# plancherb1/parallel-DDP

Measured on AMD Instinct MI355X. Metric: DDP iterations/sec (Kuka iiwa14 N=128, 8 alphas, 4 shooting segments), higher is better.
Workload: dtype f32; 1 GPU; BASELINE configs[2]: Kuka iiwa14 RBD (n=14,m=7), N=128, 8 alphas x 4 shooting segments, Euler, fp32, joint cost, T=0.5 s, WAFR example inputs + N(0,1e-3) velocity noise; problems_per_gpu=16384, problems_total=16384, hipgraph=True, cost_to_go_slots_written=all, handle_options=library defaults

## Files before the change

### parallel-ddp_amd/csrc/bp_mfma.hpp

```cpp
#pragma once

#include <hip/hip_runtime.h>

#include "ab_compact.hpp"
#include "solver_state.hpp"

#ifndef PDDP_MX_EXP
#define PDDP_MX_EXP 0
#endif

#ifndef PDDP_MX_STAGE_K
#define PDDP_MX_STAGE_K 0
#endif
#ifndef PDDP_MX_DMA_MASK
#define PDDP_MX_DMA_MASK 0
#endif
#ifndef PDDP_MX_ORDER
#define PDDP_MX_ORDER 0
#endif
#ifndef PDDP_MX_GJ
#define PDDP_MX_GJ 0
#endif

namespace pddp {
// ... 382 lines not shown
    asm volatile(
        "s_mov_b32 m0, %[l0]\n\ts_nop 0\n\tbuffer_load_dword %[v], %[dab], %[s0] offen lds\n\t"
        "s_mov_b32 m0, %[l1]\n\ts_nop 0\n\tbuffer_load_dword %[v], %[dab], %[s1] offen lds\n\t"
        "s_mov_b32 m0, %[l2]\n\ts_nop 0\n\tbuffer_load_dword %[v], %[dab], %[s2] offen lds\n\t"
        "s_mov_b32 %[keep], exec_hi\n\ts_mov_b32 exec_hi, 0\n\ts_mov_b32 m0, %[l3]\n\ts_nop 0\n\tbuffer_load_dword %[v], %[dg], %[sg] offen lds\n\t"
        "s_mov_b32 exec_hi, %[keep]"
        : [keep] "=&s"(keep)
        : [l0] "s"(l0), [l1] "s"(l0 + 4u * kMxDmaRegion), [l2] "s"(l0 + 8u * kMxDmaRegion), [l3] "s"(l0 + 12u * kMxDmaRegion), [v] "v"(lane4), [dab] "s"(dab), [dg] "s"(dg),
          [s0] "s"(s0), [s1] "s"(s1), [s2] "s"(s2), [sg] "s"(sg)
        : "memory", "m0");
#endif
    if constexpr (HQQ)
        asm volatile("s_mov_b32 m0, %[l4]\n\ts_nop 0\n\tbuffer_load_dword %[v], %[dh], %[sh] offen lds" :: [l4] "s"(l0 + 16u * kMxDmaRegion), [v] "v"(lane4), [dh] "s"(dh), [sh] "s"(sh) : "memory", "m0");
}
template <bool FS>
__device__ __forceinline__ void mx_lds_knot(MxKnotIn<float, FS, true>& k, unsigned half, unsigned aA, unsigned aB, unsigned aT, unsigned aG, int g, int c, int ub, float dt) {
    constexpr int NX = 14, NU = 7;
    typedef const float __attribute__((address_space(3))) * lptr;
    const int u0 = 2 * g, sc = mx_state<float>(c);
    const bool cx = sc < NX, cu = ub < NU, c14 = (sc == NX), g3 = g < 3;
    const lptr pA = (lptr)(size_t)(aA + half), pB = (lptr)(size_t)(aB + half), pT = (lptr)(size_t)(aT + half), pG = (lptr)(size_t)(aG + half);
    const float ta0 = pA[0], ta1 = pA[1], tb0 = pB[0], tb1 = pB[1];
    k.A0[0] = cx ? ((sc == u0) ? 1.f : ((sc == u0 + 7) ? dt : 0.f)) : 0.f;
    k.A0[1] = (cx && g3) ? ((sc == u0 + 1) ? 1.f : ((sc == u0 + 8) ? dt : 0.f)) : 0.f;
    k.A0[2] = cx ? ta0 : 0.f; k.A0[3] = (cx && g3) ? ta1 : 0.f;
    k.B1[0] = 0.f; k.B1[1] = 0.f;
    k.B1[2] = cu ? tb0 : 0.f; k.B1[3] = (cu && g3) ? tb1 : 0.f;
    if (FS) {
        const float t0 = pT[0], t1 = pT[7];
        k.BT0 = (cx && sc >= 7) ? t0 : 0.f; k.BT1 = (cx && sc >= 7 && u0 + 1 < NU) ? t1 : 0.f;
    }
    const float gx[4] = {pG[0], pG[1], pG[7], pG[8]};
    const float gu0 = pG[NX], gu1 = pG[NX + 1];
#pragma unroll
    for (int r = 0; r < 4; r++) k.CXX[r] = (c14 && (g3 || !(r & 1))) ? gx[r] : 0.f;
    k.CUX0 = c14 ? gu0 : 0.f; k.CUX1 = (c14 && u0 + 1 < NU) ? gu1 : 0.f;
    k.hx = 0.f; k.hu = 0.f;
}

__device__ __forceinline__ void mx_store_gain_pieces(const mx_u4& w, __amdgpu_buffer_rsrc_t rKT, __amdgpu_buffer_rsrc_t rdu, int lane, unsigned knot) {
    const unsigned soK = knot * (unsigned)(14 * 7 * 4), sod = knot * (unsigned)(7 * 4);
    if (lane < 24) __builtin_amdgcn_raw_buffer_store_b128(w, rKT, 16u * (unsigned)lane, soK, 0);
    else if (lane == 24) { mx_u2 h; h[0] = w[0]; h[1] = w[1]; __builtin_amdgcn_raw_buffer_store_b64(h, rKT, 384u, soK, 0); }
    else if (lane == 25) __builtin_amdgcn_raw_buffer_store_b128(w, rdu, 0u, sod, 0);
    else if (lane == 26) { mx_u3 t; t[0] = w[0]; t[1] = w[1]; t[2] = w[2]; __builtin_amdgcn_raw_buffer_store_b96(t, rdu, 16u, sod, 0); }
}
constexpr int kMxGainStores = 4, kMxCtgStores = 3;
constexpr int kMxKeepP = 1, kMxFuseSweep = 2, kMxLds = 400, kMxDmaFloats = 2 * 5 * 64 + 256 + 112;
template <typename T, bool FS, bool DIAGH, bool CAB, bool FUSE, bool HQQ = false>
__device__ void arm_mx_bp_block(T* lds, const Buffers<T>& b, const Dims& dm, int pb, int blk, T hq1, T hq2, T hr, T dt, int flags) {
    static_assert(!HQQ || DIAGH, "the compact position block rides on the diagonal-Hessian path");
    using X = Mx<T>;
    using mx4 = mx4t<T>;
    const int keepP = flags & kMxKeepP;
    const bool fuse = FUSE && blk < dm.M - 1;
    constexpr int NX = 14, NU = 7, NM = 21, SZP = NX * NX, SZAB = NX * NM, SZH = NM * NM;
    const int lane = threadIdx.x & 63, g = lane >> 4, c = lane & 15, u0 = 2 * g, sc = mx_state<T>(c);
    const int cg = X::g_of(c), cr = X::r_of(c);
    const int ub = (cr < 2) ? 2 * cg + cr : 8;
    const SolverState<T>& st = b.state[pb];
    if (st.done) return;
    const int N = dm.N, NBk = dm.NB;
    const T rho = st.rho;
    const size_t halfP = (size_t)(b.Pp - b.P), halfp = (size_t)(b.pp - b.p), knot0 = (size_t)pb * N;
    T* Pw = b.P + (st.pw ? halfP : 0) + knot0 * SZP;
    const T* Pr = b.P + (st.pw ? 0 : halfP) + knot0 * SZP;
    T* pw = b.p + (st.pw ? halfp : 0) + knot0 * NX;
    const T* pr = b.p + (st.pw ? 0 : halfp) + knot0 * NX;
    const T* AB = b.AB + knot0 * SZAB; const T* H = b.H + knot0 * SZH; const T* gg = b.g + knot0 * NM;
    T* KT = b.KT + knot0 * (NX * NU); T* du = b.du + knot0 * NU; T* ApBK = b.ApBK + knot0 * SZP; T* Bdu = b.Bdu + knot0 * NX;
    const T* dcur = b.dcur + knot0 * NX;
    const T* xc = b.xb + ((size_t)pb * 2 + st.cur) * N * NX; const T* xp2 = b.xb + ((size_t)pb * 2 + st.cur2) * N * NX;
    const bool cx = sc < NX, cu = ub < NU, c14 = (sc == NX);
    bool diag[4];
#pragma unroll
    for (int r = 0; r < 4; r++) diag[r] = (X::q_of(g, r) == c);

    int ks = NBk * (blk + 1) - 1, iterCount;
    mx4 Pa;
    if (ks == N - 1) {
        const T* Hf = H + (size_t)ks * SZH; const T* gf = gg + (size_t)ks * NM;
        Pa = mx_load_col<T>(cx ? Hf + sc * NM : gf, g, cx || c14);
        if (keepP) mx_store_col<T>(cx ? Pw + (size_t)(ks - 1) * SZP + sc * NX : pw + (size_t)(ks - 1) * NX, g, cx || c14, Pa);
        ks--; iterCount = NBk - 2;
    } else {
        iterCount = NBk - 1;
        const T* bP = Pr + (size_t)ks * SZP;
        Pa = mx_load_col<T>(bP + sc * NX, g, cx);
        if (lane < NX) {
            T dot = T(0), val = T(0);
            for (int j = 0; j < NX; j++) {
                const T pj = bP[lane + NX * j];
                dot += pj * (xc[NX * (ks + 1) + j] - xp2[NX * (ks + 1) + j]);
                val += dcur[(size_t)ks * NX + j] * pj;
            }
            lds[lane] = (dot + pr[(size_t)ks * NX + lane]) + val;
        }
        wsync();
        if (c14) {
#pragma unroll
            for (int r = 0; r < 4; r++) { const int sr = mx_state_gr(g, r); Pa[r] = (sr < NX) ? lds[sr] : T(0); }
        }
        wsync();
    }
    T dJ00 = T(0), dJ01 = T(0), dJ10 = T(0), dJ11 = T(0);
    const mx4 zero = {T(0), T(0), T(0), T(0)};
    T* ldsI = lds + 16;
// ... 317 lines not shown
```

### parallel-ddp_amd/csrc/mx_launch.hpp

```cpp
#pragma once

#include <hip/hip_runtime.h>

#include "solver_state.hpp"

namespace pddp {

template <typename T>
void launch_bp_mfma(hipStream_t s, const Buffers<T>& b, const Dims& dm, int batch, bool diag_h, T hq1, T hq2, T hr, T dt, bool keep_P, bool fuse_sweep, int ee = 0);
template <typename T>
void launch_sweep_maps(hipStream_t s, const Buffers<T>& b, const Dims& dm, int batch);

}
```

### parallel-ddp_amd/csrc/pddp_mx.hip

```cpp
#include <hip/hip_runtime.h>

#include "bp_mfma.hpp"
#include "mx_launch.hpp"

#ifdef PDDP_MX_WAVES
#define PDDP_MX_WAVES_OF(CAB, HQQ) PDDP_MX_WAVES
#else
#define PDDP_MX_WAVES_OF(CAB, HQQ) ((CAB) ? 6 : 5)
#endif

namespace pddp {

template <bool FS, bool DIAGH, bool CAB, bool FUSE, bool HQQ = false>
__global__ __launch_bounds__(64) __attribute__((amdgpu_waves_per_eu(PDDP_MX_WAVES_OF(CAB, HQQ), PDDP_MX_WAVES_OF(CAB, HQQ)))) void k_bp_mfma(Buffers<float> b, Dims dm, int batch, float hq1, float hq2, float hr, float dt, int flags) {
    __shared__ __attribute__((aligned(16))) float lds[kMxLds + kMxDmaFloats];
    const int inst = blockIdx.x;
    if (inst >= batch * dm.M) return;
    arm_mx_bp_block<float, FS, DIAGH, CAB, FUSE, HQQ>(lds, b, dm, inst / dm.M, inst % dm.M, hq1, hq2, hr, dt, flags);
}
template <bool FS, bool DIAGH, bool CAB, bool FUSE, bool HQQ = false>
__global__ __launch_bounds__(64) void k_bp_mfma_f64(Buffers<double> b, Dims dm, int batch, double hq1, double hq2, double hr, double dt, int flags) {
    __shared__ __attribute__((aligned(16))) double lds[kMxLds];
    const int inst = blockIdx.x;
    if (inst >= batch * dm.M) return;
    arm_mx_bp_block<double, FS, DIAGH, CAB, FUSE, HQQ>(lds, b, dm, inst / dm.M, inst % dm.M, hq1, hq2, hr, dt, flags);
}
__device__ __forceinline__ float mx_uniform(float v) { return __int_as_float(__builtin_amdgcn_readfirstlane(__float_as_int(v))); }
__device__ __forceinline__ double mx_uniform(double v) {
    return __hiloint2double(__builtin_amdgcn_readfirstlane(__double2hiint(v)), __builtin_amdgcn_readfirstlane(__double2loint(v)));
}
template <bool FS, bool CAB, bool FUSE, bool HQQ = false>
__global__ __launch_bounds__(64) __attribute__((amdgpu_waves_per_eu(PDDP_MX_WAVES_OF(CAB, HQQ), PDDP_MX_WAVES_OF(CAB, HQQ)))) void k_bp_mfma_pc(Buffers<float> b, Dims dm, int batch, int ee, float dt, int flags) {
    __shared__ __attribute__((aligned(16))) float lds[kMxLds + kMxDmaFloats];
    const int inst = blockIdx.x;
    if (inst >= batch * dm.M) return;
    float hq1, hq2, hr;
    cost_diag_weights_at<float>(b.cwt, ee, inst / dm.M, hq1, hq2, hr);
    arm_mx_bp_block<float, FS, true, CAB, FUSE, HQQ>(lds, b, dm, inst / dm.M, inst % dm.M, mx_uniform(hq1), mx_uniform(hq2), mx_uniform(hr), dt, flags);
}
template <bool FS, bool CAB, bool FUSE, bool HQQ = false>
__global__ __launch_bounds__(64) void k_bp_mfma_f64_pc(Buffers<double> b, Dims dm, int batch, int ee, double dt, int flags) {
    __shared__ __attribute__((aligned(16))) double lds[kMxLds];
    const int inst = blockIdx.x;
    if (inst >= batch * dm.M) return;
    double hq1, hq2, hr;
    cost_diag_weights_at<double>(b.cwt, ee, inst / dm.M, hq1, hq2, hr);
    arm_mx_bp_block<double, FS, true, CAB, FUSE, HQQ>(lds, b, dm, inst / dm.M, inst % dm.M, mx_uniform(hq1), mx_uniform(hq2), mx_uniform(hr), dt, flags);
}
template <bool FS, bool DIAGH, bool CAB, bool FUSE, bool HQQ = false>
static void launch_one(hipStream_t s, unsigned n, const Buffers<float>& b, const Dims& dm, int batch, float hq1, float hq2, float hr, float dt, int kp, int ee) {
    if constexpr (DIAGH) { if (b.cwt) { hipLaunchKernelGGL((k_bp_mfma_pc<FS, CAB, FUSE, HQQ>), dim3(n), dim3(64), 0, s, b, dm, batch, ee, dt, kp); return; } }
    hipLaunchKernelGGL((k_bp_mfma<FS, DIAGH, CAB, FUSE, HQQ>), dim3(n), dim3(64), 0, s, b, dm, batch, hq1, hq2, hr, dt, kp);
}
template <bool FS, bool DIAGH, bool CAB, bool FUSE, bool HQQ = false>
static void launch_one(hipStream_t s, unsigned n, const Buffers<double>& b, const Dims& dm, int batch, double hq1, double hq2, double hr, double dt, int kp, int ee) {
    if constexpr (DIAGH) { if (b.cwt) { hipLaunchKernelGGL((k_bp_mfma_f64_pc<FS, CAB, FUSE, HQQ>), dim3(n), dim3(64), 0, s, b, dm, batch, ee, dt, kp); return; } }
    hipLaunchKernelGGL((k_bp_mfma_f64<FS, DIAGH, CAB, FUSE, HQQ>), dim3(n), dim3(64), 0, s, b, dm, batch, hq1, hq2, hr, dt, kp);
}

template <typename T>
void launch_bp_mfma(hipStream_t s, const Buffers<T>& b, const Dims& dm, int batch, bool diag_h, T hq1, T hq2, T hr, T dt, bool keep_P, bool fuse_sweep, int ee) {
    const unsigned n = (unsigned)batch * dm.M;
    const int kp = (keep_P ? kMxKeepP : 0) | ((fuse_sweep && b.segmap) ? kMxFuseSweep : 0);
    const bool cab = b.ABc != nullptr && diag_h;
#define PDDP_MX_LAUNCH(FS, DH, CB, FU) launch_one<FS, DH, CB, FU>(s, n, b, dm, batch, hq1, hq2, hr, dt, kp, ee)
    const bool fu = (kp & kMxFuseSweep) != 0;
    if (cab && b.Hc) {
#define PDDP_MX_LAUNCH_Q(FS, FU) launch_one<FS, true, true, FU, true>(s, n, b, dm, batch, hq1, hq2, hr, dt, kp, ee)
        if (dm.M > 1) { if (fu) PDDP_MX_LAUNCH_Q(true, true); else PDDP_MX_LAUNCH_Q(true, false); }
        else PDDP_MX_LAUNCH_Q(false, false);
#undef PDDP_MX_LAUNCH_Q
        return;
    }
    if (dm.M > 1) {
        if (cab) { if (fu) PDDP_MX_LAUNCH(true, true, true, true); else PDDP_MX_LAUNCH(true, true, true, false); }
        else if (diag_h) { if (fu) PDDP_MX_LAUNCH(true, true, false, true); else PDDP_MX_LAUNCH(true, true, false, false); }
        else { if (fu) PDDP_MX_LAUNCH(true, false, false, true); else PDDP_MX_LAUNCH(true, false, false, false); }
    } else {
        if (cab) PDDP_MX_LAUNCH(false, true, true, false);
        else if (diag_h) PDDP_MX_LAUNCH(false, true, false, false);
        else PDDP_MX_LAUNCH(false, false, false, false);
    }
#undef PDDP_MX_LAUNCH
}
template void launch_bp_mfma<float>(hipStream_t, const Buffers<float>&, const Dims&, int, bool, float, float, float, float, bool, bool, int);
template void launch_bp_mfma<double>(hipStream_t, const Buffers<double>&, const Dims&, int, bool, double, double, double, double, bool, bool, int);

template <typename T, int PER>
__global__ __launch_bounds__(64) void k_sweep_maps(Buffers<T> b, Dims dm, int batch) {
    constexpr int NX = 14, W = 64 / PER;
    const int lane = threadIdx.x % W, pb = blockIdx.x * PER + threadIdx.x / W;
    if (pb >= batch) return;
    const SolverState<T>& st = b.state[pb];
    if (st.done) return;
    for (int i = 0; i < dm.M; i++) if (b.err[(size_t)pb * dm.M + i]) return;
    const int N = dm.N, NBk = dm.NB, l = lane < NX ? lane : NX - 1;
    const T* xcur = b.xb + ((size_t)pb * 2 + st.cur) * N * NX; const T* dcur = b.dcur + (size_t)pb * N * NX;
    T es = T(0), et = T(0);
    if (dm.M == 4) {
        constexpr int S = 3;
        T ph[S][NX + 1], dk[S], base[S];
#pragma unroll
        for (int sgm = 0; sgm < S; sgm++) {
            const T* o = b.segmap + ((size_t)pb * 4 + sgm) * 256;
            const int k = (sgm + 1) * NBk - 1;
#pragma unroll
            for (int cc = 0; cc <= NX; cc++) ph[sgm][cc] = o[cc * 16 + l];
            dk[sgm] = dcur[(size_t)k * NX + l]; base[sgm] = xcur[(size_t)(k + 1) * NX + l];
        }
#pragma unroll
        for (int sgm = 0; sgm < S; sgm++) {
            const int k = (sgm + 1) * NBk - 1;
            T ns = ph[sgm][NX], nt = dk[sgm];
#pragma unroll
            for (int cc = 0; cc < NX; cc++) { ns = Mx<T>::fma(ph[sgm][cc], __shfl(es, cc, W), ns); nt = Mx<T>::fma(ph[sgm][cc], __shfl(et, cc, W), nt); }
            es = ns; et = nt;
            if (lane < NX) for (int a = 0; a < dm.A; a++) b.xs[(((size_t)pb * dm.A + a) * N + k + 1) * NX + lane] = base[sgm] + (et - b.alpha[a] * es);
        }
        return;
    }
    for (int sgm = 0; sgm < dm.M - 1; sgm++) {
        const T* o = b.segmap + ((size_t)pb * dm.M + sgm) * 256;
        const int k = (sgm + 1) * NBk - 1;
        T ns = o[14 * 16 + l], nt = dcur[(size_t)k * NX + l];
#pragma unroll
        for (int cc = 0; cc < NX; cc++) {
            const T ph = o[cc * 16 + l];
            ns = Mx<T>::fma(ph, __shfl(es, cc, W), ns); nt = Mx<T>::fma(ph, __shfl(et, cc, W), nt);
        }
        es = ns; et = nt;
        if (lane < NX) {
            const T base = xcur[(size_t)(k + 1) * NX + lane];
            for (int a = 0; a < dm.A; a++) b.xs[(((size_t)pb * dm.A + a) * N + k + 1) * NX + lane] = base + (et - b.alpha[a] * es);
        }
    }
}
template <typename T>
void launch_sweep_maps(hipStream_t s, const Buffers<T>& b, const Dims& dm, int batch) {
    if (batch >= 2048) hipLaunchKernelGGL((k_sweep_maps<T, 4>), dim3((unsigned)((batch + 3) / 4)), dim3(64), 0, s, b, dm, batch);
// ... 7 lines not shown
```

### parallel-ddp_amd/csrc/solver_impl.hpp

```cpp
#pragma once
#include "solver_base.hpp"
#include "kernels.hpp"
#include "handle_setup.hpp"
#include "slots.hpp"
#include "cost_table.hpp"
#include "diag_cost_table.hpp"
#include "goal_traj_table.hpp"
#include "mpc_slots.hpp"
#include "mpc_record.hpp"
#include "tl_launch.hpp"
#include "mx_launch.hpp"

using namespace pddp;

template <typename P, int INTEG, typename T>
struct Solver : SolverBase {
    static constexpr int NX = P::NX, NU = P::NU, NM = NX + NU, NP = P::NPOS;
    Buffers<T> b{};
    MpcBuffers<T> mb{};
    T* d_xActual = nullptr; T* d_goal_in = nullptr; int* d_shift = nullptr;
    unsigned char* d_mpc_out = nullptr;
    PinnedBuf h_state;
    PinnedBuf h_stage;
    Dims dm{};
    SolverParams sp{};
    CostWeights<T> cw{};
    T dt{};
    std::map<std::string, std::pair<void*, size_t>> arrays;
    std::vector<DeviceBuf> allocs;
    template <typename Mem> int reserve(MemBuf<Mem>& buf, size_t bytes, const char* what, size_t min_cap = 0) {
        if (buf.holds(bytes)) return 0;
        if (buf.ptr) HIPCHK(hipStreamSynchronize(stream));
        return buf.reserve(bytes, min_cap) ? 0 : fail(Mem::kFailCode, what);
    }
    KernelPlan plan;
    void resolve_plan() { plan = make_kernel_plan(cfg, PlantTraits{P::PLANT, NX, NU, P::kScalarPlugin, P::kPluginCost}, sizeof(T) == 4, tl_variant); }
    int tl_variant = -1;
    T tl_grav = T(0);
    void derive_tl_model(const ArmModel<T>& hm) {
        ArmTlModel<T> m;
        tl_variant = -1;
        if (arm_tl_model_from_tables(m, hm))
            for (int v = 0; v < 2; v++) if (arm_tl_models_equal(m, arm_tl_builtin<T>(v))) tl_variant = v;
        tl_grav = hm.grav;
    }
    void derive_tl_model(const EmptyModel&) {}
    void drop_graph() override { if (graph) { hipGraphExecDestroy(graph); graph = nullptr; graph_mode = -1; } if (graph_n) { hipGraphExecDestroy(graph_n); graph_n = nullptr; } }
    int ab_view(int to_compact) override {
        if constexpr (P::PLANT == 4) {
            if (b.ABc) { launch_abc_convert<T>(stream, b, (int)(cfg.batch * cfg.N), cfg.N, dt, to_compact); HIPCHK(hipGetLastError()); HIPCHK(hipStreamSynchronize(stream)); }
        }
        return 0;
    }
    int ab_keep_reference_layout() override {
        if (!b.ABc) return 0;
        int rc = ab_view(0);
        b.ABc = nullptr; b.Hc = nullptr; drop_graph();
        return rc;
    }
    int h_view() override {
        if constexpr (P::PLANT == 4) {
            if (b.Hc) {
                hipLaunchKernelGGL((k_hc_expand<T>), dim3((cfg.batch * cfg.N + 63) / 64), dim3(64), 0, stream, b, (int)(cfg.batch * cfg.N), cfg.N, hw[1], hw[2]);
                HIPCHK(hipGetLastError()); HIPCHK(hipStreamSynchronize(stream));
            }
        }
        return 0;
    }
    int cand_view(int to_records) override {
        if constexpr (P::PLANT != 4) {
            if (b.xw && plan.cf_fp_staged) {
                const dim3 g((unsigned)(((size_t)cfg.batch * cfg.N * cfg.A + 255) / 256));
                if (to_records) hipLaunchKernelGGL((k_cand_to_xw<P, T>), g, dim3(256), 0, stream, b, dm, (int)cfg.batch);
                else hipLaunchKernelGGL((k_xw_to_cand<P, T>), g, dim3(256), 0, stream, b, dm, (int)cfg.batch);
                HIPCHK(hipGetLastError()); HIPCHK(hipStreamSynchronize(stream));
            }
        }
        cand_stale = false;
        return 0;
    }
    int reference_views(int what) override {
        if ((what & 1) && cfg.M > 1) { int rc = ab_view(0); if (rc) return rc; }
        hipLaunchKernelGGL((k_reference_views<P, T>), dim3(cfg.N, cfg.batch), dim3(64), 0, stream, b, dm, what);
        HIPCHK(hipGetLastError()); HIPCHK(hipStreamSynchronize(stream));
        if (what & 1) fs_vars_stale = false;
        if (what & 2) cand_stale = false;
        return 0;
    }
    int model_changed() override {
        typename P::Model hm;
        HIPCHK(hipMemcpy(&hm, b.model, sizeof(hm), hipMemcpyDeviceToHost));
        derive_tl_model(hm);
        resolve_plan();
        drop_graph();
        return 0;
    }
    bool mpc_used = false;
    bool lean_ctg_ran = false;
    bool keep_all_ctg() const { return !cfg.boundary_cost_to_go_only || cfg.mpc_mode || mpc_used; }
    hipGraphExec_t graph = nullptr;
    int graph_mode = -1;
    size_t fp_lds = 0;

    ~Solver() override {
        drop_graph();
        for (hipEvent_t e : trace_ev) hipEventDestroy(e);
        for (hipEvent_t e : slots_ev) if (e) hipEventDestroy(e);
        delete intake;
        if (stream && !intake_of) hipStreamDestroy(stream);
    }
    void register_model(void* dmodel, const ArmModel<T>&) {
        arrays["model_I"] = {dmodel, sizeof(T) * kArmNB * 36};
        arrays["model_F"] = {(char*)dmodel + offsetof(ArmModel<T>, F), sizeof(T) * kArmNB * 16};
    }
    void register_model(void*, const EmptyModel&) {}
    template <typename U> int alloc(const char* name, U** out, size_t count) {
        DeviceBuf blk;
        if (!blk.reserve(count * sizeof(U))) return fail(PDDP_ENOMEM, std::string("hipMalloc failed for ") + name);
        if (hipMemset(blk.ptr, 0, count * sizeof(U)) != hipSuccess) return fail(PDDP_ENODEVICE, "hipMemset failed");
        arrays[name] = {blk.ptr, count * sizeof(U)}; *out = blk.template as<U>();
        allocs.push_back(std::move(blk));
        return 0;
    }
    int init() override {
        const pddp_config& c = cfg;
        int ndev = 0;
        if (hipGetDeviceCount(&ndev) != hipSuccess || ndev <= c.device)
            return fail(PDDP_ENODEVICE, "no HIP device available: libpddp has no CPU fallback");
        HIPCHK(hipSetDevice(c.device));
#ifdef PDDP_REF_PLANT_FILE
        if constexpr (P::PLANT == 5) { const std::string complaint = ref_plugin_setup<T>(c.N); if (!complaint.empty()) return fail(PDDP_EINVAL, complaint); }
#endif
        if constexpr (P::PLANT == 5) {
            if (!scalar_plugin_qdd_is_dynamics<P, T>())
                return fail(PDDP_EINVAL, "plant 5: the plug-in's gradient routine returns a qdd that differs from its dynamics routine at the same state; the kernel families build the "
                                         "integrators' stage states from either one, so the two have to be the same numbers (call the dynamics routine inside the gradient routine)");
        }
        if (intake_of) stream = intake_of->stream;
        else HIPCHK(hipStreamCreateWithFlags(&stream, hipStreamNonBlocking));
        dm.N = c.N; dm.M = c.M; dm.A = c.A; dm.NB = c.N / c.M;
        cap_batch = c.batch;
        sp = solver_params_of(c); cw = cost_weights_of<T, P::PLANT>(c); dt = time_step<T>(c);
        const size_t B = c.batch, N = c.N, A = c.A, M = c.M;
        int rc = for_each_array<NX, NU>(c, b, mb, arrays, [this](const char* name, auto** out, size_t count) { return alloc(name, out, count); });
        if (rc) return rc;
        const MpcInputRun in = mpc_input_run(sizeof(T), NX, B);
        if ((rc = alloc("mpc_in", &d_xActual, in.elems))) return rc;
        d_goal_in = mpc_at<T>(d_xActual, in.goal); d_shift = mpc_at<int>(d_xActual, in.shift);
        arrays["xActual"] = {d_xActual, in.x_bytes}; arrays["shift"] = {d_shift, in.shift_bytes};
        std::vector<T> al(A);
        alpha_table(c, al.data());
        HIPCHK(hipMemcpy(b.alpha, al.data(), A * sizeof(T), hipMemcpyHostToDevice));
        typename P::Model hm; fill_model(hm, c);
// ... 147 lines not shown
            break;
        }
        if constexpr (P::PLANT != 4) { if (L.cand_to_xw && b.xw) hipLaunchKernelGGL((k_cand_to_xw<P, T>), dim3((unsigned)(((size_t)B * cfg.N * cfg.A + 255) / 256)), dim3(256), 0, s, b, dm, (int)B); }
    }
    T hw[3] = {T(0), T(0), T(0)};
    void note_setup_weights() { const bool ee = cfg.ee_cost != 0; hw[0] = ee ? cw.Q_xEE : cw.Q1; hw[1] = ee ? cw.Q_xdEE : cw.Q2; hw[2] = ee ? cw.R_EE : cw.R; }
    void launch_nis(hipStream_t s, int mode, int part = -1) {
        const unsigned B = cfg.batch;
        if (part == 0) return;
        note_setup_weights();
        switch (plan.nis) {
        case kNisTl:
            if constexpr (P::PLANT == 4) launch_nis_tl<T>(s, tl_variant, b, dm, cw, dt, tl_grav, mode, (int)B);
            break;
        case kNisTl7:
            if constexpr (P::PLANT == 4) launch_nis_tl7<T>(s, tl_variant, b, dm, cw, dt, tl_grav, mode, (int)B);
            break;
        case kNisLg:
            if constexpr (P::PLANT == 4) {
                if (cfg.ee_cost) hipLaunchKernelGGL((k_nis_lg<T, true>), dim3((cfg.N + 31) / 32, B), dim3(256), 0, s, b, dm, cw, dt, mode);
                else hipLaunchKernelGGL((k_nis_lg<T>), dim3((cfg.N + 31) / 32, B), dim3(256), 0, s, b, dm, cw, dt, mode);
            }
            break;
        case kNisTs:
            if constexpr (P::PLANT != 4) with_cost_plant([&](auto pl) { using Q = decltype(pl); hipLaunchKernelGGL((k_nis_ts<Q, INTEG, T>), dim3((B * cfg.N + 63) / 64), dim3(64), 0, s, b, dm, cw, dt, mode, (int)B); });
            break;
        case kNisKb:
            if constexpr (P::PLANT != 4 && P::NX + P::NU <= 16 && INTEG == 3 && P::kScalarPlugin) {
                const int units = (int)(B * cfg.N);
                with_cost_plant([&](auto pl) {
                    using Q = decltype(pl);
                    if (plan.kb_nis == 16) hipLaunchKernelGGL((k_nis_kb<Q, T, 16>), dim3((units + 15) / 16), dim3(64), 0, s, b, dm, cw, dt, mode, (int)B);
                    else if (plan.kb_nis == 20) hipLaunchKernelGGL((k_nis_kb<Q, T, 20>), dim3((units + 19) / 20), dim3(64), 0, s, b, dm, cw, dt, mode, (int)B);
                    else if (plan.kb_nis == 64 && sizeof(T) == 4) hipLaunchKernelGGL((k_nis_kb<Q, T, sizeof(T) == 4 ? 64 : 16>), dim3((units + 63) / 64), dim3(64), 0, s, b, dm, cw, dt, mode, (int)B);
                    else hipLaunchKernelGGL((k_nis_kb<Q, T, 32>), dim3((units + 31) / 32), dim3(64), 0, s, b, dm, cw, dt, mode, (int)B);
                });
            }
            break;
        case kNisGl:
            if constexpr (P::PLANT != 4 && P::NX + P::NU <= 16) {
                with_cost_plant([&](auto pl) {
                    using Q = decltype(pl);
                    if (plan.gl_nis8) hipLaunchKernelGGL((k_nis_gl<Q, INTEG, T, 8>), dim3((B * cfg.N + 7) / 8), dim3(64), 0, s, b, dm, cw, dt, mode, (int)B);
                    else hipLaunchKernelGGL((k_nis_gl<Q, INTEG, T, 16>), dim3((B * cfg.N + 3) / 4), dim3(64), 0, s, b, dm, cw, dt, mode, (int)B);
                });
            }
            break;
        case kNisCoop:
            if constexpr (P::PLANT == 4) { if (b.cwt) { hipLaunchKernelGGL((k_nis<P, INTEG, T, true>), dim3(cfg.N, B), dim3(64), 0, s, b, dm, cw, dt, mode); break; } }
            with_cost_plant([&](auto pl) { using Q = decltype(pl); hipLaunchKernelGGL((k_nis<Q, INTEG, T>), dim3(cfg.N, B), dim3(64), 0, s, b, dm, cw, dt, mode); });
            break;
        }
    }
    void launch_bp(hipStream_t s, int store_candidates, bool fused_hook = false) {
        const unsigned B = cfg.batch;
        switch (plan.bp) {
        case kBpMfma:
            if constexpr (P::PLANT == 4) {
                const bool ee = cfg.ee_cost != 0;
                const bool diag_h = !h_overridden && (!ee || b.Hc != nullptr);
                launch_bp_mfma<T>(s, b, dm, (int)B, diag_h, hw[0], hw[1], hw[2], dt, keep_all_ctg() || store_candidates,
                                  plan.sweep_fused && (!store_candidates || fused_hook), ee ? 1 : 0);
            }
            break;
        case kBpLg:
            if constexpr (P::PLANT == 4) hipLaunchKernelGGL((k_bp_lg<T>), dim3((B * cfg.M + kLgPerWave - 1) / kLgPerWave), dim3(64), 0, s, b, dm, (int)B);
            break;
        case kBpTs:
            if constexpr (P::PLANT != 4) hipLaunchKernelGGL((k_bp_ts<P, T>), dim3((B * cfg.M + 63) / 64), dim3(64), 0, s, b, dm, (int)B);
            break;
        case kBpMq:
            if constexpr (P::PLANT != 4 && P::NX == 12 && P::NU == 4) {
                const bool fu = plan.mq_fused && (!store_candidates || fused_hook);
                const bool dh = !P::kPluginCost && !h_overridden;
                if (dh && fu) with_weight_plant([&](auto pl) { using Q = decltype(pl); hipLaunchKernelGGL((k_bp_mq<Q, T, true, true>), dim3(B * cfg.M), dim3(64), 0, s, b, dm, cw, (int)B); });
                else if (dh) with_weight_plant([&](auto pl) { using Q = decltype(pl); hipLaunchKernelGGL((k_bp_mq<Q, T, true>), dim3(B * cfg.M), dim3(64), 0, s, b, dm, cw, (int)B); });
                else if (fu) hipLaunchKernelGGL((k_bp_mq<P, T, false, true>), dim3(B * cfg.M), dim3(64), 0, s, b, dm, cw, (int)B);
                else hipLaunchKernelGGL((k_bp_mq<P, T, false>), dim3(B * cfg.M), dim3(64), 0, s, b, dm, cw, (int)B);
            }
            break;
        case kBpCl:
            if constexpr (P::PLANT != 4 && P::NX == 12 && P::NU == 4)
                with_weight_plant([&](auto pl) { using Q = decltype(pl); hipLaunchKernelGGL((k_bp_cl<Q, T>), dim3((B * cfg.M + 3) / 4), dim3(64), 0, s, b, dm, cw, (int)B, (!P::kPluginCost && !h_overridden) ? 1 : 0); });
            break;
        case kBpGl:
            if constexpr (P::PLANT != 4 && P::NX + P::NU <= 16) {
                if (plan.gl_bp32) hipLaunchKernelGGL((k_bp_gl<P, T, 32>), dim3((B * cfg.M + 1) / 2), dim3(64), 0, s, b, dm, (int)B);
                else hipLaunchKernelGGL((k_bp_gl<P, T, 16>), dim3((B * cfg.M + 3) / 4), dim3(64), 0, s, b, dm, (int)B);
            }
            break;
        case kBpWide: hipLaunchKernelGGL((k_bp_wide<P, T>), dim3(cfg.M, B), dim3(256), 0, s, b, dm); break;
        case kBpCoop: hipLaunchKernelGGL((k_bp<P, T>), dim3(cfg.M, B), dim3(64), 0, s, b, dm); break;
        }
    }
    void launch_sweep(hipStream_t s, int only = -1, int store_candidates = 0, int part = -1) {
        const unsigned B = cfg.batch;
        if (only < 0 || only == PDDP_PHASE_BP) launch_bp(s, store_candidates);
        if (only < 0 || only == PDDP_PHASE_FP) launch_fp(s, store_candidates ? kFpHook : part == 0 ? kFpSweepOnly : part == 1 ? kFpRolloutsOnly : kFpProduction);
        if ((only < 0 || only == PDDP_PHASE_LS) && !(plan.ls_in_rollouts && !store_candidates)) {
            if (plan.ls_many) hipLaunchKernelGGL((k_ls_many<T>), dim3((unsigned)((B + 63) / 64)), dim3(64), 0, s, b, dm, sp, bench_mode, (int)B);
            else hipLaunchKernelGGL((k_ls<T>), dim3(B), dim3(64), 0, s, b, dm, sp, bench_mode);
        }
        if (only < 0 || only == PDDP_PHASE_NIS) launch_nis(s, 0, part);
    }
    int time_kernels(int sweeps, float* ms, char* names, int name_stride) override {
        const char* nm[6];
        plan_kernel_names(plan, cfg, nm);
        static const int phase_of[6] = {PDDP_PHASE_BP, PDDP_PHASE_FP, PDDP_PHASE_FP, PDDP_PHASE_LS, PDDP_PHASE_NIS, PDDP_PHASE_NIS};
        const int part_of[6] = {-1, 0, plan.maps_in_rollouts ? -1 : 1, -1, 0, 1};
        HIPCHK(hipStreamSynchronize(stream));
        note_sweeps_enqueued();
        if (int erc = need_events(7 * (size_t)sweeps)) return erc;
        for (int i = 0; i < sweeps; i++) {
            HIPCHK(hipEventRecord(trace_ev[7 * i], stream));
            for (int k = 0; k < 6; k++) { if (nm[k][0]) launch_sweep(stream, phase_of[k], 0, part_of[k]); HIPCHK(hipEventRecord(trace_ev[7 * i + k + 1], stream)); }
        }
        HIPCHK(hipGetLastError());
        HIPCHK(hipStreamSynchronize(stream));
        for (int k = 0; k < 6; k++) {
            double sum = 0;
            for (int i = 0; i < sweeps; i++) { float t = 0; HIPCHK(hipEventElapsedTime(&t, trace_ev[7 * i + k], trace_ev[7 * i + k + 1])); sum += t; }
            ms[k] = nm[k][0] ? (float)(sum / sweeps) : 0.f;
            if (names) { std::strncpy(names + (size_t)k * name_stride, nm[k], name_stride - 1); names[(size_t)k * name_stride + name_stride - 1] = 0; }
        }
        return 0;
    }
    static constexpr int kGraphUnroll = 4;
    hipGraphExec_t graph_n = nullptr;
    int capture_sweeps(int count, hipGraphExec_t* out) {
        hipGraph_t gr;
        HIPCHK(hipStreamBeginCapture(stream, hipStreamCaptureModeThreadLocal));
        for (int i = 0; i < count; i++) launch_sweep(stream);
        {
            const hipError_t le = hipGetLastError(), ce = hipStreamEndCapture(stream, &gr);
            if (le != hipSuccess || ce != hipSuccess) {
                if (ce == hipSuccess && gr) hipGraphDestroy(gr);
                return fail(PDDP_ENODEVICE, std::string("sweep capture failed: ") + hipGetErrorString(le != hipSuccess ? le : ce));
            }
        }
        HIPCHK(hipGraphInstantiate(out, gr, nullptr, nullptr, 0));
        HIPCHK(hipGraphDestroy(gr));
        return 0;
    }
    void note_sweeps_enqueued() {
        if (plan.sweep_fused || plan.mq_fused) fs_vars_stale = true;
        if (plan.cf_fp && plan.cf_fp_staged) cand_stale = true;
    }
    int iterate(int sweeps) override {
        if (plan.bp_mfma && !keep_all_ctg()) lean_ctg_ran = true;
        if (sweeps > 0) note_sweeps_enqueued();
        if (cfg.use_graph) {
            if (!graph || graph_mode != bench_mode + 2 * sp.max_iter) {
                if (graph) { hipGraphExecDestroy(graph); graph = nullptr; }
                if (graph_n) { hipGraphExecDestroy(graph_n); graph_n = nullptr; }
                int rc = capture_sweeps(1, &graph);
                if (rc) return rc;
                graph_mode = bench_mode + 2 * sp.max_iter;
            }
            int left = sweeps;
            if (left >= kGraphUnroll && (size_t)cfg.batch * cfg.N <= 65536) {
                if (!graph_n) { int rc = capture_sweeps(kGraphUnroll, &graph_n); if (rc) return rc; }
                for (; left >= kGraphUnroll; left -= kGraphUnroll) HIPCHK(hipGraphLaunch(graph_n, stream));
            }
            for (int i = 0; i < left; i++) HIPCHK(hipGraphLaunch(graph, stream));
        } else {
            for (int i = 0; i < sweeps; i++) launch_sweep(stream);
        }
        HIPCHK(hipGetLastError());
        return 0;
    }
    std::vector<hipEvent_t> trace_ev;
    int need_events(size_t n) { while (trace_ev.size() < n) { hipEvent_t e; HIPCHK(hipEventCreate(&e)); trace_ev.push_back(e); } return 0; }
    int iterate_traced(int sweeps, double* phase_ms, int first_sweep, int stride) override {
        if (sweeps > 0) note_sweeps_enqueued();
        if (int erc = need_events(6 * (size_t)sweeps)) return erc;
        static const int phase_of[5] = {PDDP_PHASE_BP, PDDP_PHASE_FP, PDDP_PHASE_FP, PDDP_PHASE_LS, PDDP_PHASE_NIS};
        const bool own_sweep = !plan.maps_in_rollouts;
        const int part_of[5] = {-1, 0, own_sweep ? 1 : -1, -1, -1};
        for (int i = 0; i < sweeps; i++) {
            HIPCHK(hipEventRecord(trace_ev[6 * i], stream));
            for (int k = 0; k < 5; k++) { if (k != 1 || own_sweep) launch_sweep(stream, phase_of[k], 0, part_of[k]); HIPCHK(hipEventRecord(trace_ev[6 * i + k + 1], stream)); }
        }
        HIPCHK(hipGetLastError());
        HIPCHK(hipStreamSynchronize(stream));
        for (int i = 0; i < sweeps; i++) {
            if (first_sweep + i >= stride) continue;
            float ms[5];
            for (int k = 0; k < 5; k++) HIPCHK(hipEventElapsedTime(&ms[k], trace_ev[6 * i + k], trace_ev[6 * i + k + 1]));
            if (!own_sweep) ms[1] = 0.f;
            const size_t o = (size_t)first_sweep + i;
            phase_ms[0 * (size_t)stride + o] = ms[0]; phase_ms[1 * (size_t)stride + o] = (double)ms[1] + ms[2]; phase_ms[2 * (size_t)stride + o] = ms[3];
            phase_ms[3 * (size_t)stride + o] = ms[4]; phase_ms[4 * (size_t)stride + o] = ms[1];
        }
        return 0;
    }
    int sync() override { HIPCHK(hipStreamSynchronize(stream)); return 0; }
    int set_cost(double Q1, double Q2, double R, double QF1, double QF2) override {
        HIPCHK(hipStreamSynchronize(stream));
        cfg.Q1 = Q1; cfg.Q2 = Q2; cfg.R = R; cfg.QF1 = QF1; cfg.QF2 = QF2;
        cw = cost_weights_of<T, P::PLANT>(cfg);
        drop_graph();
        return fill_cost_table();
    }
    int set_cost_ee(const double* v) override {
        if (!cfg.ee_cost) return fail(PDDP_EINVAL, "pddp_set_cost_ee: the handle was not created with ee_cost = 1");
        HIPCHK(hipStreamSynchronize(stream));
        cfg.Q_EE1 = v[0]; cfg.Q_EE2 = v[1]; cfg.QF_EE1 = v[2]; cfg.QF_EE2 = v[3]; cfg.R_EE = v[4]; cfg.Q_xEE = v[5]; cfg.QF_xEE = v[6]; cfg.Q_xdEE = v[7]; cfg.QF_xdEE = v[8];
        cw = cost_weights_of<T, P::PLANT>(cfg);
        drop_graph();
        return fill_cost_table();
    }
    DeviceBuf d_cwt;
    T* cwt_rows() const { return d_cwt.template as<T>(); }
    std::vector<T> cwt_stage;
    int cost_record_size() const override { return P::PLANT == 4 && !P::kPluginCost ? cost_record_len(cfg.ee_cost) : 0; }
    int cwt_move_rows(int count, const int* idx, int rec, bool to_device) {
        hipError_t e = hipSuccess;
        for_each_slot_run(count, idx, [&](int first, int len) {
            T* h = cwt_stage.data() + (size_t)first * rec; T* d = cwt_rows() + (size_t)idx[first] * rec;
            if (e == hipSuccess) e = to_device ? hipMemcpyAsync(d, h, (size_t)len * rec * sizeof(T), hipMemcpyHostToDevice, stream) : hipMemcpyAsync(h, d, (size_t)len * rec * sizeof(T), hipMemcpyDeviceToHost, stream);
        });
        if (e != hipSuccess) return fail(PDDP_ENODEVICE, std::string("cost table: transfer of rows failed: ") + hipGetErrorString(e));
        HIPCHK(hipStreamSynchronize(stream));
        return 0;
    }
    int cwt_upload_rows(int count, const int* idx, int rec) { return cwt_move_rows(count, idx, rec, true); }
    int cwt_download_rows(int count, const int* idx, int rec) { return cwt_move_rows(count, idx, rec, false); }
    int cwt_fill_rows(int rows, int rec, const T* record) {
        cwt_stage.resize((size_t)rows * rec);
        for (int i = 0; i < rows; i++) std::memcpy(cwt_stage.data() + (size_t)i * rec, record, rec * sizeof(T));
        HIPCHK(hipMemcpyAsync(cwt_rows(), cwt_stage.data(), cwt_stage.size() * sizeof(T), hipMemcpyHostToDevice, stream));
        HIPCHK(hipStreamSynchronize(stream));
        return 0;
    }
// ... 717 lines not shown
```

### parallel-ddp_amd/csrc/solver_state.hpp

```cpp
#pragma once

#include <cstddef>

#include "pddp_common.hpp"

namespace pddp {

template <typename T>
struct SolverState {
    T rho, drho, prevJ, dJ, z;
    int iter;
    int alphaIndex;
    int ignore_defect;
    int accepted;
    int done;
    int cur, cur2;
    int bp_retries;
    int pw;
    int took_step;
    int win_pending;
};

struct SolverParams {
    int max_iter;
// ... 42 lines not shown
    s.drho = tmax(s.drho * T(kRhoFactor), T(kRhoFactor));
    s.rho = tmin(s.rho * s.drho, T(kRhoMax));
}
template <typename T> PDDP_HD void rho_decrease(SolverState<T>& s) {
    s.drho = tmin(s.drho / T(kRhoFactor), T(1.0 / kRhoFactor));
    s.rho = tmax(s.rho * s.drho, T(kRhoMin));
}

template <typename T>
PDDP_HD void line_search_accept(SolverState<T>& st, const SolverParams& sp, const Dims& dm, int any_bp_err, const T* alpha,
                                const T* J, const T* dmax, T* dJexp, T* Jout, int* alphaOut) {
    if (st.done) return;
    st.win_pending = 0;
    if (any_bp_err) {
        rho_increase(st);
        st.accepted = -1;
        st.bp_retries++;
        if ((st.rho == T(kRhoMax) && !sp.ignore_max_rho_exit) || st.bp_retries > 200) st.done = 3;
        return;
    }
    for (int i = 1; i < dm.M; i++) { dJexp[0] += dJexp[2 * i]; dJexp[1] += dJexp[2 * i + 1]; }
    T dJ = -1, z = 0;
    int aidx = st.alphaIndex;
    for (int i = 0; i < dm.A; i++) {
        const T cdJ = st.prevJ - J[i];
        const bool JFlag = cdJ >= T(0) && cdJ > dJ;
        const T cz = cdJ / (alpha[i] * dJexp[0] + T(0.5) * alpha[i] * alpha[i] * dJexp[1]);
        const bool zFlag = T(sp.exp_red_min) < cz && cz < T(sp.exp_red_max);
        const bool dFlag = (dm.M == 1 || st.ignore_defect) ? true : dmax[i] < T(sp.max_defect);
        if (JFlag && zFlag && dFlag) {
            if (dmax[i] < T(sp.max_defect)) st.ignore_defect = 0;
            aidx = i; dJ = cdJ; z = cz;
        }
    }
    st.z = z;
    st.cur2 = st.cur;
    if (dJ < T(0)) {
        rho_increase(st);
        st.alphaIndex = 0; alphaOut[st.iter] = -1; Jout[st.iter] = st.prevJ;
        st.accepted = 0; st.dJ = dJ;
        if (st.rho == T(kRhoMax) && !sp.ignore_max_rho_exit) { st.done = 3; return; }
    } else {
        rho_decrease(st);
        dJ = dJ / st.prevJ; st.prevJ = J[aidx];
        st.alphaIndex = aidx; alphaOut[st.iter] = aidx; Jout[st.iter] = J[aidx];
        if (aidx > 0) st.took_step = 1;
        st.accepted = 1; st.dJ = dJ; st.win_pending = 1;
        st.cur = 1 - st.cur;
        if (dJ < T(sp.tol_cost)) { st.done = 1; return; }
    }
    if (st.iter == sp.max_iter) st.done = 2; else { st.iter += 1; st.pw ^= 1; }
}

}
```

Before: 7.605 million DDP iterations/s.

## Skip cost-to-go stores in early sweeps unless the problem may exit soon

Adds a lean mode in which the MFMA backward pass drops the full per-knot cost-to-go (P) writes for every sweep except the last two in a batch. A problem still gets them when its state shows it could terminate within two iterations (near max_iter or near max rho). Separate lean and non-lean HIP graphs are captured so the lean sweeps run first and the kept sweeps run at the tail. This cuts global-memory store traffic in the backward pass, but it relies on a conservative exit predictor and adds complexity to graph capture.

```diff
diff --git a/parallel-ddp_amd/csrc/bp_mfma.hpp b/parallel-ddp_amd/csrc/bp_mfma.hpp
--- a/parallel-ddp_amd/csrc/bp_mfma.hpp
+++ b/parallel-ddp_amd/csrc/bp_mfma.hpp
@@ -458,7 +458,7 @@
     static_assert(!HQQ || DIAGH, "the compact position block rides on the diagonal-Hessian path");
     using X = Mx<T>;
     using mx4 = mx4t<T>;
-    const int keepP = flags & kMxKeepP;
+    const int keepP = (flags & kMxKeepP) || ((flags & kMxLeanIfRunning) && may_exit_within_two(b.state[pb], flags));
     const bool fuse = FUSE && blk < dm.M - 1;
     constexpr int NX = 14, NU = 7, NM = 21, SZP = NX * NX, SZAB = NX * NM, SZH = NM * NM;
     const int lane = threadIdx.x & 63, g = lane >> 4, c = lane & 15, u0 = 2 * g, sc = mx_state<T>(c);
diff --git a/parallel-ddp_amd/csrc/mx_launch.hpp b/parallel-ddp_amd/csrc/mx_launch.hpp
--- a/parallel-ddp_amd/csrc/mx_launch.hpp
+++ b/parallel-ddp_amd/csrc/mx_launch.hpp
@@ -7,7 +7,8 @@
 namespace pddp {
 
 template <typename T>
-void launch_bp_mfma(hipStream_t s, const Buffers<T>& b, const Dims& dm, int batch, bool diag_h, T hq1, T hq2, T hr, T dt, bool keep_P, bool fuse_sweep, int ee = 0);
+void launch_bp_mfma(hipStream_t s, const Buffers<T>& b, const Dims& dm, int batch, bool diag_h, T hq1, T hq2, T hr, T dt, bool keep_P, bool fuse_sweep, int ee = 0,
+                    const SolverParams* lean_if_running = nullptr);
 template <typename T>
 void launch_sweep_maps(hipStream_t s, const Buffers<T>& b, const Dims& dm, int batch);
 
diff --git a/parallel-ddp_amd/csrc/pddp_mx.hip b/parallel-ddp_amd/csrc/pddp_mx.hip
--- a/parallel-ddp_amd/csrc/pddp_mx.hip
+++ b/parallel-ddp_amd/csrc/pddp_mx.hip
@@ -59,9 +59,10 @@
 }
 
 template <typename T>
-void launch_bp_mfma(hipStream_t s, const Buffers<T>& b, const Dims& dm, int batch, bool diag_h, T hq1, T hq2, T hr, T dt, bool keep_P, bool fuse_sweep, int ee) {
+void launch_bp_mfma(hipStream_t s, const Buffers<T>& b, const Dims& dm, int batch, bool diag_h, T hq1, T hq2, T hr, T dt, bool keep_P, bool fuse_sweep, int ee, const SolverParams* lean_if_running) {
     const unsigned n = (unsigned)batch * dm.M;
-    const int kp = (keep_P ? kMxKeepP : 0) | ((fuse_sweep && b.segmap) ? kMxFuseSweep : 0);
+    int kp = (keep_P ? kMxKeepP : 0) | ((fuse_sweep && b.segmap) ? kMxFuseSweep : 0);
+    if (!keep_P && lean_if_running) kp |= kMxLeanIfRunning | (lean_if_running->ignore_max_rho_exit ? 0 : kMxMaxRhoExit) | lean_flags_max_iter(lean_if_running->max_iter);
     const bool cab = b.ABc != nullptr && diag_h;
 #define PDDP_MX_LAUNCH(FS, DH, CB, FU) launch_one<FS, DH, CB, FU>(s, n, b, dm, batch, hq1, hq2, hr, dt, kp, ee)
     const bool fu = (kp & kMxFuseSweep) != 0;
@@ -83,8 +84,8 @@
     }
 #undef PDDP_MX_LAUNCH
 }
-template void launch_bp_mfma<float>(hipStream_t, const Buffers<float>&, const Dims&, int, bool, float, float, float, float, bool, bool, int);
-template void launch_bp_mfma<double>(hipStream_t, const Buffers<double>&, const Dims&, int, bool, double, double, double, double, bool, bool, int);
+template void launch_bp_mfma<float>(hipStream_t, const Buffers<float>&, const Dims&, int, bool, float, float, float, float, bool, bool, int, const SolverParams*);
+template void launch_bp_mfma<double>(hipStream_t, const Buffers<double>&, const Dims&, int, bool, double, double, double, double, bool, bool, int, const SolverParams*);
 
 template <typename T, int PER>
 __global__ __launch_bounds__(64) void k_sweep_maps(Buffers<T> b, Dims dm, int batch) {
diff --git a/parallel-ddp_amd/csrc/solver_impl.hpp b/parallel-ddp_amd/csrc/solver_impl.hpp
--- a/parallel-ddp_amd/csrc/solver_impl.hpp
+++ b/parallel-ddp_amd/csrc/solver_impl.hpp
@@ -45,7 +45,10 @@
         tl_grav = hm.grav;
     }
     void derive_tl_model(const EmptyModel&) {}
-    void drop_graph() override { if (graph) { hipGraphExecDestroy(graph); graph = nullptr; graph_mode = -1; } if (graph_n) { hipGraphExecDestroy(graph_n); graph_n = nullptr; } }
+    void drop_graph() override {
+        for (hipGraphExec_t* g : {&graph, &graph_lean, &graph_n, &graph_n_lean}) if (*g) { hipGraphExecDestroy(*g); *g = nullptr; }
+        graph_mode = -1;
+    }
     int ab_view(int to_compact) override {
         if constexpr (P::PLANT == 4) {
             if (b.ABc) { launch_abc_convert<T>(stream, b, (int)(cfg.batch * cfg.N), cfg.N, dt, to_compact); HIPCHK(hipGetLastError()); HIPCHK(hipStreamSynchronize(stream)); }
@@ -98,7 +101,13 @@
     bool mpc_used = false;
     bool lean_ctg_ran = false;
     bool keep_all_ctg() const { return !cfg.boundary_cost_to_go_only || cfg.mpc_mode || mpc_used; }
-    hipGraphExec_t graph = nullptr;
+    static constexpr int kKeepSweeps = 2;
+    bool split_sweeps() const {
+        const T w[] = {cw.Q1, cw.Q2, cw.R, cw.QF1, cw.QF2, cw.Q_EE1, cw.Q_EE2, cw.QF_EE1, cw.QF_EE2, cw.R_EE, cw.Q_xEE, cw.QF_xEE, cw.Q_xdEE, cw.QF_xdEE};
+        for (T v : w) if (!(v >= T(0))) return false;
+        return plan.bp_mfma && keep_all_ctg() && !(sp.tol_cost > 0.0) && !b.cwt;
+    }
+    hipGraphExec_t graph = nullptr, graph_lean = nullptr;
     int graph_mode = -1;
     size_t fp_lds = 0;
 
@@ -352,15 +361,15 @@
             break;
         }
     }
-    void launch_bp(hipStream_t s, int store_candidates, bool fused_hook = false) {
+    void launch_bp(hipStream_t s, int store_candidates, bool fused_hook = false, bool lean = false) {
         const unsigned B = cfg.batch;
         switch (plan.bp) {
         case kBpMfma:
             if constexpr (P::PLANT == 4) {
                 const bool ee = cfg.ee_cost != 0;
                 const bool diag_h = !h_overridden && (!ee || b.Hc != nullptr);
-                launch_bp_mfma<T>(s, b, dm, (int)B, diag_h, hw[0], hw[1], hw[2], dt, keep_all_ctg() || store_candidates,
-                                  plan.sweep_fused && (!store_candidates || fused_hook), ee ? 1 : 0);
+                launch_bp_mfma<T>(s, b, dm, (int)B, diag_h, hw[0], hw[1], hw[2], dt, (keep_all_ctg() && !lean) || store_candidates,
+                                  plan.sweep_fused && (!store_candidates || fused_hook), ee ? 1 : 0, lean ? &sp : nullptr);
             }
             break;
         case kBpLg:
@@ -393,9 +402,9 @@
         case kBpCoop: hipLaunchKernelGGL((k_bp<P, T>), dim3(cfg.M, B), dim3(64), 0, s, b, dm); break;
         }
     }
-    void launch_sweep(hipStream_t s, int only = -1, int store_candidates = 0, int part = -1) {
+    void launch_sweep(hipStream_t s, int only = -1, int store_candidates = 0, int part = -1, bool lean = false) {
         const unsigned B = cfg.batch;
-        if (only < 0 || only == PDDP_PHASE_BP) launch_bp(s, store_candidates);
+        if (only < 0 || only == PDDP_PHASE_BP) launch_bp(s, store_candidates, false, lean);
         if (only < 0 || only == PDDP_PHASE_FP) launch_fp(s, store_candidates ? kFpHook : part == 0 ? kFpSweepOnly : part == 1 ? kFpRolloutsOnly : kFpProduction);
         if ((only < 0 || only == PDDP_PHASE_LS) && !(plan.ls_in_rollouts && !store_candidates)) {
             if (plan.ls_many) hipLaunchKernelGGL((k_ls_many<T>), dim3((unsigned)((B + 63) / 64)), dim3(64), 0, s, b, dm, sp, bench_mode, (int)B);
@@ -412,8 +421,9 @@
         note_sweeps_enqueued();
         if (int erc = need_events(7 * (size_t)sweeps)) return erc;
         for (int i = 0; i < sweeps; i++) {
+            const bool lean = split_sweeps() && i + kKeepSweeps < sweeps;
             HIPCHK(hipEventRecord(trace_ev[7 * i], stream));
-            for (int k = 0; k < 6; k++) { if (nm[k][0]) launch_sweep(stream, phase_of[k], 0, part_of[k]); HIPCHK(hipEventRecord(trace_ev[7 * i + k + 1], stream)); }
+            for (int k = 0; k < 6; k++) { if (nm[k][0]) launch_sweep(stream, phase_of[k], 0, part_of[k], lean); HIPCHK(hipEventRecord(trace_ev[7 * i + k + 1], stream)); }
         }
         HIPCHK(hipGetLastError());
         HIPCHK(hipStreamSynchronize(stream));
@@ -426,11 +436,11 @@
         return 0;
     }
     static constexpr int kGraphUnroll = 4;
-    hipGraphExec_t graph_n = nullptr;
-    int capture_sweeps(int count, hipGraphExec_t* out) {
+    hipGraphExec_t graph_n = nullptr, graph_n_lean = nullptr;
+    int capture_sweeps(int count, int lean, hipGraphExec_t* out) {
         hipGraph_t gr;
         HIPCHK(hipStreamBeginCapture(stream, hipStreamCaptureModeThreadLocal));
-        for (int i = 0; i < count; i++) launch_sweep(stream);
+        for (int i = 0; i < count; i++) launch_sweep(stream, -1, 0, -1, i < lean);
         {
             const hipError_t le = hipGetLastError(), ce = hipStreamEndCapture(stream, &gr);
             if (le != hipSuccess || ce != hipSuccess) {
@@ -449,22 +459,32 @@
     int iterate(int sweeps) override {
         if (plan.bp_mfma && !keep_all_ctg()) lean_ctg_ran = true;
         if (sweeps > 0) note_sweeps_enqueued();
-        if (cfg.use_graph) {
-            if (!graph || graph_mode != bench_mode + 2 * sp.max_iter) {
-                if (graph) { hipGraphExecDestroy(graph); graph = nullptr; }
-                if (graph_n) { hipGraphExecDestroy(graph_n); graph_n = nullptr; }
-                int rc = capture_sweeps(1, &graph);
+        const bool split = split_sweeps();
+        if (sweeps > 0 && cfg.use_graph) {
+            const int key = bench_mode + 2 * sp.max_iter + (split ? 1 << 30 : 0);
+            if (!graph || graph_mode != key) {
+                drop_graph();
+                int rc = capture_sweeps(1, 0, &graph);
                 if (rc) return rc;
-                graph_mode = bench_mode + 2 * sp.max_iter;
-            }
-            int left = sweeps;
-            if (left >= kGraphUnroll && (size_t)cfg.batch * cfg.N <= 65536) {
-                if (!graph_n) { int rc = capture_sweeps(kGraphUnroll, &graph_n); if (rc) return rc; }
-                for (; left >= kGraphUnroll; left -= kGraphUnroll) HIPCHK(hipGraphLaunch(graph_n, stream));
-            }
-            for (int i = 0; i < left; i++) HIPCHK(hipGraphLaunch(graph, stream));
+                graph_mode = key;
+            }
+            auto need = [&](hipGraphExec_t* g, int count, int lean) { return *g ? 0 : capture_sweeps(count, lean, g); };
+            const bool unroll = sweeps >= kGraphUnroll && (size_t)cfg.batch * cfg.N <= 65536;
+            const int tail = unroll ? kGraphUnroll : sweeps < kKeepSweeps ? sweeps : kKeepSweeps;
+            int front = sweeps - tail;
+            if (split && front > 0) { if (int rc = need(&graph_lean, 1, 1)) return rc; }
+            hipGraphExec_t one = split ? graph_lean : graph;
+            if (unroll) {
+                if (int rc = need(&graph_n, kGraphUnroll, split ? kGraphUnroll - kKeepSweeps : 0)) return rc;
+                if (split && front >= kGraphUnroll) { if (int rc = need(&graph_n_lean, kGraphUnroll, kGraphUnroll)) return rc; }
+                hipGraphExec_t four = split ? graph_n_lean : graph_n;
+                for (; front >= kGraphUnroll; front -= kGraphUnroll) HIPCHK(hipGraphLaunch(four, stream));
+            }
+            for (; front > 0; front--) HIPCHK(hipGraphLaunch(one, stream));
+            if (unroll) HIPCHK(hipGraphLaunch(graph_n, stream));
+            else for (int i = 0; i < tail; i++) HIPCHK(hipGraphLaunch(graph, stream));
         } else {
-            for (int i = 0; i < sweeps; i++) launch_sweep(stream);
+            for (int i = 0; i < sweeps; i++) launch_sweep(stream, -1, 0, -1, split && i + kKeepSweeps < sweeps);
         }
         HIPCHK(hipGetLastError());
         return 0;
@@ -478,8 +498,9 @@
         const bool own_sweep = !plan.maps_in_rollouts;
         const int part_of[5] = {-1, 0, own_sweep ? 1 : -1, -1, -1};
         for (int i = 0; i < sweeps; i++) {
+            const bool lean = split_sweeps() && i + kKeepSweeps < sweeps;
             HIPCHK(hipEventRecord(trace_ev[6 * i], stream));
-            for (int k = 0; k < 5; k++) { if (k != 1 || own_sweep) launch_sweep(stream, phase_of[k], 0, part_of[k]); HIPCHK(hipEventRecord(trace_ev[6 * i + k + 1], stream)); }
+            for (int k = 0; k < 5; k++) { if (k != 1 || own_sweep) launch_sweep(stream, phase_of[k], 0, part_of[k], lean); HIPCHK(hipEventRecord(trace_ev[6 * i + k + 1], stream)); }
         }
         HIPCHK(hipGetLastError());
         HIPCHK(hipStreamSynchronize(stream));
diff --git a/parallel-ddp_amd/csrc/solver_state.hpp b/parallel-ddp_amd/csrc/solver_state.hpp
--- a/parallel-ddp_amd/csrc/solver_state.hpp
+++ b/parallel-ddp_amd/csrc/solver_state.hpp
@@ -118,4 +118,13 @@
     if (st.iter == sp.max_iter) st.done = 2; else { st.iter += 1; st.pw ^= 1; }
 }
 
+constexpr int kMxLeanIfRunning = 4, kMxMaxRhoExit = 8, kMxMaxIterShift = 8;
+PDDP_HD constexpr int lean_flags_max_iter(int max_iter) { return (max_iter < (1 << 22) ? max_iter : (1 << 22) - 1) << kMxMaxIterShift; }
+template <typename T>
+PDDP_HD bool may_exit_within_two(const SolverState<T>& st, int flags) {
+    if (st.iter >= (flags >> kMxMaxIterShift) - 1) return true;
+    if (flags & kMxMaxRhoExit) { SolverState<T> t = st; rho_increase(t); rho_increase(t); if (t.rho == T(kRhoMax)) return true; }
+    return false;
 }
+
+}
```

After: 8.126 million DDP iterations/s, median of 6. 1.07x the previous value.
